# ray-project/anyscale-workshop-nyc-2023

Measured on NVIDIA H100. Metric: generated tokens/sec (and prompts/sec) FLAN-T5-base 512->128, higher is better.
Workload: dtype bf16

## Files before the change

### anyscale_workshop_nyc_2023_b200/_lib.py

```python
from __future__ import annotations

import ctypes as C
import os
import subprocess
from pathlib import Path

_HERE = Path(__file__).resolve().parent
LIB_PATH = _HERE / "libb200t5.so"
LIB_PATHS = {"bf16": LIB_PATH, "fp16": _HERE / "libb200t5_f16.so"}
CSRC = _HERE / "csrc"

OK, EINVAL, ENODEV, ECUDA, ESTATE, ENOMEM = 0, -1, -2, -3, -4, -5
DTYPE_BF16, DTYPE_F16, DTYPE_F32 = 0, 1, 2


class Config(C.Structure):
    _fields_ = [
        ("vocab_size", C.c_int32),
        ("d_model", C.c_int32),
        ("d_kv", C.c_int32),
        ("d_ff", C.c_int32),
        ("num_heads", C.c_int32),
        ("num_layers", C.c_int32),
        ("num_decoder_layers", C.c_int32),
# ... 3 lines not shown
        ("pad_token_id", C.c_int32),
        ("eos_token_id", C.c_int32),
        ("decoder_start_token_id", C.c_int32),
        ("is_gated_gelu", C.c_int32),
        ("scale_decoder_outputs", C.c_int32),
    ]


class GenParams(C.Structure):
    _fields_ = [
        ("max_new_tokens", C.c_int32),
        ("min_new_tokens", C.c_int32),
        ("eos_token_id", C.c_int32),
        ("pad_token_id", C.c_int32),
        ("decoder_start_token_id", C.c_int32),
        ("poll_interval", C.c_int32),
    ]


class Stats(C.Structure):
    _fields_ = [
        ("encoder_ms", C.c_float),
        ("decode_ms", C.c_float),
        ("decode_steps", C.c_int32),
        ("kernel_launches", C.c_int64),
        ("decode_algo_bytes", C.c_double),
        ("encoder_flops", C.c_double),
        ("xattn_kernel", C.c_int32),
        ("row_chains", C.c_int32),
    ]


_vp, _i, _i64p, _i32p = C.c_void_p, C.c_int, C.c_void_p, C.c_void_p

SIGNATURES = {
    "b200t5_create": (_i, [C.POINTER(Config), _i, C.POINTER(_vp)]),
    "b200t5_set_weight": (_i, [_vp, C.c_char_p, _vp, _i, C.POINTER(C.c_int64), _i]),
    "b200t5_finalize": (_i, [_vp]),
    "b200t5_destroy": (_i, [_vp]),
    "b200t5_last_error": (C.c_char_p, [_vp]),
    "b200t5_last_global_error": (C.c_char_p, []),
    "b200t5_generate": (_i, [_vp, _i64p, _i64p, _i, _i, C.POINTER(GenParams), _i64p, _i32p, _vp]),
    "b200t5_generate_host": (_i, [_vp, _i64p, _i64p, _i, _i, C.POINTER(GenParams), _i64p, _i32p]),
    "b200t5_generate_stream": (_i, [_vp, _i64p, _i64p, C.c_int64, _i, C.POINTER(GenParams), _i, _i, _i64p, _i32p]),
    "b200t5_get_stats": (_i, [_vp, C.POINTER(Stats)]),
    "b200t5_bench_cross_attn": (_i, [_vp, _i, _i, C.POINTER(C.c_float), C.POINTER(C.c_double), _vp]),
    "b200t5_set_option": (_i, [_vp, C.c_char_p, _i]),
    "b200t5_get_xattn_profile": (_i, [_vp, C.POINTER(C.c_double), C.POINTER(C.c_int64), C.POINTER(C.c_double), C.POINTER(C.c_double), C.POINTER(C.c_double)]),
    "b200t5_test_lm_argmax": (_i, [_i, _vp, _vp, _i, _i, _i, _i, _i, _i, _vp, _vp]),
    "b200t5_encode": (_i, [_vp, _i64p, _i64p, _i, _i, _vp, _vp]),
    "b200t5_decode_logits": (_i, [_vp, _i64p, _i64p, _i, _i, _i64p, _i, _vp, _vp]),
    "b200t5_relative_bucket": (_i, [_i, _i, _i, _i]),
    "b200t5_test_gemm": (_i, [_i, _vp, _vp, _vp, _i, _i, _i, _i, _i, _i, _vp]),
    "b200t5_test_gemm_splitk": (_i, [_i, _vp, _vp, _vp, _i, _i, _i, _i, _i, _i, _i, _vp, _i, _i, _vp]),
    "b200t5_test_ffo": (_i, [_i, _vp, _vp, _vp, _i, _i, _i, _i, _i, _i, _vp]),
    "b200t5_test_rmsnorm": (_i, [_i, _vp, _vp, _vp, _i, _i, C.c_float, _vp]),
    "b200t5_test_attn_decode": (_i, [_i, _i, _vp, _vp, _vp, _vp, _i, _i, _i, _vp, _vp, _i, _vp, _vp]),
    "b200t5_test_encoder_attn": (_i, [_i, _vp, _vp, _vp, _vp, _vp, _i, _i, _i, _i, _vp]),
    "b200t5_test_geglu": (_i, [_i, _vp, _vp, _vp, C.c_int64, _i, _vp]),
    "b200t5_version": (C.c_char_p, []),
}

_libs = {}


def build(force: bool = False) -> Path:
    for path in LIB_PATHS.values():
        if force and path.exists():
            path.unlink()
    proc = subprocess.run(["make", "-j2", "-C", str(CSRC)], capture_output=True, text=True)
    if proc.returncode != 0 or not all(path.exists() for path in LIB_PATHS.values()):
        raise RuntimeError(f"building libb200t5.so / libb200t5_f16.so failed:\n{proc.stdout}\n{proc.stderr}")
    return LIB_PATH


def load(flavour: str = "bf16") -> C.CDLL:
    if flavour in _libs:
        return _libs[flavour]
    path = LIB_PATHS[flavour]
    if not path.exists():
        raise RuntimeError(
            f"{path} is missing: run `make -C {CSRC}` (or __graft_entry__.build()). "
            "There is no CPU or PyTorch fallback for the CUDA path."
        )
    lib = C.CDLL(str(path), mode=getattr(os, "RTLD_NOW", 2))
    for name, (res, args) in SIGNATURES.items():
        try:
            fn = getattr(lib, name)
        except AttributeError as e:
            raise RuntimeError(f"{path.name} does not export {name}") from e
        fn.restype = res
        fn.argtypes = args
    _libs[flavour] = lib
    return lib


def last_error(handle=None, lib=None) -> str:
    lib = lib or load()
    msg = lib.b200t5_last_error(handle) if handle else lib.b200t5_last_global_error()
    return (msg or b"").decode("utf-8", "replace")


class B200T5Error(RuntimeError):
    def __init__(self, code: int, msg: str):
        super().__init__(f"libb200t5 error {code}: {msg}")
        self.code = code
# ... 6 lines not shown
```

### anyscale_workshop_nyc_2023_b200/csrc/b200t5.cu

```cuda
#include <cuda.h>
#include <cuda_bf16.h>
#include <cuda_fp16.h>
#include <cuda_runtime.h>
#include <math.h>
#include <stdarg.h>
#include <stdio.h>
#include <string.h>

#include <map>
#include <memory>
#include <string>
#include <vector>

#include "../../include/b200t5.h"
#include "attention_decode.cuh"
#include "attention_cross_stream.cuh"
#include "attention_encoder.cuh"
#include "elementwise.cuh"
#include "gemm.cuh"
#include "gemm_splitk.cuh"
#include "gemm_2cta.cuh"

using namespace b200;

// ... 198 lines not shown
  cudaGraphExec_t gexec8 = nullptr;
  long long g_eos = -1, g_pad = -1;
  int g_min_new = -1;
  long long* h_ids = nullptr;
  long long* h_mask = nullptr;
  long long* h_out = nullptr;
  int* h_len = nullptr;
  DecodeState* h_state = nullptr;
  ~Plan() {
    if (gexec) cudaGraphExecDestroy(gexec);
    if (graph) cudaGraphDestroy(graph);
    if (gexec8) cudaGraphExecDestroy(gexec8);
    if (graph8) cudaGraphDestroy(graph8);
    if (h_ids) cudaFreeHost(h_ids);
    if (h_mask) cudaFreeHost(h_mask);
    if (h_out) cudaFreeHost(h_out);
    if (h_len) cudaFreeHost(h_len);
    if (h_state) cudaFreeHost(h_state);
    if (h_cu) cudaFreeHost(h_cu);
    if (h_unf) cudaFreeHost(h_unf);
    if (h_admit) cudaFreeHost(h_admit);
  }
};

struct b200t5_ctx {
  Cfg c;
  int device = 0;
  int num_sms = 132;
  bool finalized = false;
  int ffo_k = 0;
  char err[512] = "";
  std::map<std::string, std::unique_ptr<DevBuf>> raw;
  std::map<std::string, std::unique_ptr<DevBuf>> raw_f32;
  std::map<std::string, std::vector<int64_t>> raw_shape;
  DevBuf shared, lm_head, enc_final_ln, dec_final_ln, enc_relbias, dec_relbias, wcrosskv;
  CUtensorMap tm_lm, tm_crosskv, tm2_crosskv;
  std::vector<float> enc_relbias_h, dec_relbias_h;
  std::vector<EncLayerW> enc;
  std::vector<DecLayerW> dec;
  std::unique_ptr<Plan> plan;
  cudaStream_t cap_stream = nullptr, exec_stream = nullptr, enc_stream = nullptr;
  cudaEvent_t enc_done_ev = nullptr, admitted_ev = nullptr;
  bool admit_overlap = true;
  cudaEvent_t ev[4] = {nullptr, nullptr, nullptr, nullptr};
  bool ev_valid = false;
  int pow_mode = 0;
  bool use_pdl = true;
  GeluLut gelu_lut{nullptr, 0, 0};
  struct SkChoice {
    int bn, split;
  };
  bool pack_rows = true;
  bool use_2cta = true;
  bool self_block = true;
  int xattn_mode = 2;
  int xs_stages = 5;
  bool xs_late_pdl = true;
  bool xs_l2_prefetch = false;
  bool xattn_serialize = false;
  std::vector<cudaEvent_t> xattn_ev;
  bool profile_xattn = false;
  int small_prio = 0;
  bool sk_on = true;
  int sk_stages64 = 0, sk_stages128 = 0;
  SkChoice sk_qkv{64, 2}, sk_proj{64, 4}, sk_wi{128, 2}, sk_ffo{64, 4};
  int chains_override = 0;
  cudaStream_t chain_streams[kMaxChains] = {};
  cudaEvent_t chain_ev[kMaxChains + 1] = {};
  int64_t launches = 0;
  int last_steps = 0;
  double last_decode_bytes = 0, last_enc_flops = 0;
};

static int fail(b200t5_ctx* h, int code, const char* fmt, ...) {
  char buf[512];
  va_list ap;
  va_start(ap, fmt);
  vsnprintf(buf, sizeof(buf), fmt, ap);
  va_end(ap);
  if (h) snprintf(h->err, sizeof(h->err), "%s", buf);
  snprintf(g_err, sizeof(g_err), "%s", buf);
  return code;
}

static int check_device(b200t5_ctx* h, int device) {
  int n = 0;
  cudaError_t e = cudaGetDeviceCount(&n);
  if (e != cudaSuccess || n <= 0)
    return fail(h, B200T5_ENODEV, "no CUDA device available (%s); libb200t5 has no CPU fallback",
                e == cudaSuccess ? "count=0" : cudaGetErrorString(e));
  if (device < 0 || device >= n) return fail(h, B200T5_EINVAL, "device %d out of range (%d devices)", device, n);
  cudaDeviceProp p;
  CU_OK(h, cudaGetDeviceProperties(&p, device));
  if (p.major != 9)
    return fail(h, B200T5_ENODEV, "device %d is sm_%d%d; libb200t5 is built for sm_90a only", device, p.major, p.minor);
  CU_OK(h, cudaSetDevice(device));
  return p.multiProcessorCount;
}

extern "C" int b200t5_relative_bucket(int rel, int bidirectional, int num_buckets, int max_distance) {
  int ret = 0, n;
  if (bidirectional) {
    num_buckets /= 2;
    if (rel > 0) ret += num_buckets;
    n = rel < 0 ? -rel : rel;
  } else {
    n = rel < 0 ? -rel : 0;
  }
  const int max_exact = num_buckets / 2;
  if (n < max_exact) return ret + n;
  const float ratio = static_cast<float>(n) / static_cast<float>(max_exact);
  const float denom = static_cast<float>(log(static_cast<double>(max_distance) / static_cast<double>(max_exact)));
  const float scaled = logf(ratio) / denom * static_cast<float>(num_buckets - max_exact);
  int large = max_exact + static_cast<int>(scaled);
  if (large > num_buckets - 1) large = num_buckets - 1;
  return ret + large;
}

static cudaError_t run_gemm(b200t5_ctx* h, const GemmOp& g, const void* ep, cudaStream_t s, bool pdl = false) {
  h->launches++;
  switch (g.kind) {
    case G_STORE256:
      return launch_gemm<256, EpiStore>(g.tmA, g.tmB, g.M, g.N, g.K, g.m_fastest, *static_cast<const EpiStore::Params*>(ep), h->num_sms, s, pdl);
    case G_RES256:
      return launch_gemm<256, EpiResidual>(g.tmA, g.tmB, g.M, g.N, g.K, g.m_fastest, *static_cast<const EpiResidual::Params*>(ep), h->num_sms, s, pdl);
    case G_GEGLU256:
      return launch_gemm<256, EpiGeglu>(g.tmA, g.tmB, g.M, g.N, g.K, g.m_fastest, *static_cast<const EpiGeglu::Params*>(ep), h->num_sms, s, pdl);
    case G_CROSSKV256:
      return launch_gemm<256, EpiCrossKV>(g.tmA, g.tmB, g.M, g.N, g.K, g.m_fastest, *static_cast<const EpiCrossKV::Params*>(ep), h->num_sms, s, pdl);
    case G_QKVDEC64:
      return launch_gemm<64, EpiQkvDecode>(g.tmA, g.tmB, g.M, g.N, g.K, g.m_fastest, *static_cast<const EpiQkvDecode::Params*>(ep), h->num_sms, s, pdl);
    case G_STORE32:
      return launch_gemm<32, EpiStore>(g.tmA, g.tmB, g.M, g.N, g.K, g.m_fastest, *static_cast<const EpiStore::Params*>(ep), h->num_sms, s, pdl);
    case G_RES32:
      return launch_gemm<32, EpiResidual>(g.tmA, g.tmB, g.M, g.N, g.K, g.m_fastest, *static_cast<const EpiResidual::Params*>(ep), h->num_sms, s, pdl);
    case G_GEGLU64:
      return launch_gemm<64, EpiGeglu>(g.tmA, g.tmB, g.M, g.N, g.K, g.m_fastest, *static_cast<const EpiGeglu::Params*>(ep), h->num_sms, s, pdl);
    case G_ARGMAX128:
      return launch_gemm<128, EpiArgmax>(g.tmA, g.tmB, g.M, g.N, g.K, g.m_fastest, *static_cast<const EpiArgmax::Params*>(ep), h->num_sms, s, pdl);
    case G_LOGITS128:
      return launch_gemm<128, EpiStoreF32>(g.tmA, g.tmB, g.M, g.N, g.K, g.m_fastest, *static_cast<const EpiStoreF32::Params*>(ep), h->num_sms, s, pdl);
  }
  return cudaErrorInvalidValue;
}

template <class Epi>
static cudaError_t run_gemm_2cta(b200t5_ctx* h, const CUtensorMap& tmA, const CUtensorMap& tmB, int M, int N, int K,
                                 const typename Epi::Params& ep, cudaStream_t s) {
  h->launches++;
  return launch_gemm_2cta<Epi>(tmA, tmB, M, N, K, ep, h->num_sms, s);
}

template <class Epi>
static cudaError_t run_gemm_sk(b200t5_ctx* h, const b200t5_ctx::SkChoice& ch, const CUtensorMap& tmA,
                               const CUtensorMap& tmB, int M, int N, int K, const typename Epi::Params& ep,
                               cudaStream_t s, bool pdl) {
  h->launches++;
  const int split = splitk_factor(K, ch.split);
  if (ch.bn == 128) return launch_gemm_splitk<128, Epi>(tmA, tmB, M, N, K, split, ep, s, pdl, 0, h->sk_stages128);
  return launch_gemm_splitk<64, Epi>(tmA, tmB, M, N, K, split, ep, s, pdl, 0, h->sk_stages64);
}

static cudaError_t run_ffo_2cta(b200t5_ctx* h, const CUtensorMap& tmA, const CUtensorMap& tmB, int M, int N,
                                const EpiResidual::Params& ep, cudaStream_t s) {
  h->launches++;
  return launch_gemm_2cta<EpiResidual, B200T5_F16 != 0>(tmA, tmB, M, N, h->ffo_k, ep, h->num_sms, s, B200T5_F16 ? h->ffo_k / 64 : 0);
}
static cudaError_t run_ffo_sk(b200t5_ctx* h, const b200t5_ctx::SkChoice& ch, const CUtensorMap& tmA, const CUtensorMap& tmB,
                              int M, int N, const EpiResidual::Params& ep, cudaStream_t s, bool pdl) {
  h->launches++;
  constexpr bool tf = B200T5_F16 != 0;
  const int split = splitk_factor(h->ffo_k, ch.split, tf ? kBK / 2 : kBK);
  const int akb = tf ? h->ffo_k / 64 : 0;
  if (ch.bn == 128) return launch_gemm_splitk<128, EpiResidual, tf>(tmA, tmB, M, N, h->ffo_k, split, ep, s, pdl, akb, h->sk_stages128);
  return launch_gemm_splitk<64, EpiResidual, tf>(tmA, tmB, M, N, h->ffo_k, split, ep, s, pdl, akb, h->sk_stages64);
}

static cudaError_t run_rmsnorm(b200t5_ctx* h, const res_t* x, const act_t* w, act_t* y, int M, int d, float eps,
                               cudaStream_t s, bool pdl = false) {
  if (h) h->launches++;
  const int wpb = 8;
  const int grid = (M + wpb - 1) / wpb;
  if (d <= 1024) return launch_kernel(rmsnorm_kernel<4>, dim3(grid), dim3(wpb * 32), 0, s, pdl, x, w, y, M, d, eps);
  if (d <= 4096) return launch_kernel(rmsnorm_kernel<16>, dim3(grid), dim3(wpb * 32), 0, s, pdl, x, w, y, M, d, eps);
  return cudaErrorInvalidValue;
}

static cudaError_t init_kernel_attrs() {
  cudaError_t e;
#define PREP(BN, EPI)                         \
  if ((e = prepare_gemm<BN, EPI>()) != cudaSuccess) return e;
  PREP(256, EpiStore) PREP(256, EpiResidual) PREP(256, EpiGeglu) PREP(256, EpiCrossKV) PREP(64, EpiQkvDecode)
  PREP(32, EpiStore) PREP(32, EpiResidual) PREP(64, EpiGeglu) PREP(128, EpiArgmax) PREP(128, EpiStoreF32)
  PREP(64, EpiStore) PREP(128, EpiStore)
#undef PREP
  if ((e = prepare_gemm_2cta<EpiStore>()) != cudaSuccess) return e;
  if ((e = prepare_gemm_2cta<EpiResidual>()) != cudaSuccess) return e;
  if ((e = prepare_gemm_2cta<EpiGeglu>()) != cudaSuccess) return e;
  if ((e = prepare_gemm_2cta<EpiCrossKV>()) != cudaSuccess) return e;
#define PREPSK(BN, EPI) \
  if ((e = prepare_gemm_splitk<BN, EPI>()) != cudaSuccess) return e;
  PREPSK(64, EpiStore) PREPSK(128, EpiStore) PREPSK(64, EpiResidual) PREPSK(128, EpiResidual)
  PREPSK(64, EpiQkvDecode) PREPSK(128, EpiQkvDecode) PREPSK(64, EpiGeglu) PREPSK(128, EpiGeglu)
#undef PREPSK
  if ((e = prepare_gemm_2cta<EpiResidual, B200T5_F16 != 0>()) != cudaSuccess) return e;
  if ((e = prepare_gemm_splitk<64, EpiResidual, B200T5_F16 != 0>()) != cudaSuccess) return e;
  if ((e = prepare_gemm_splitk<128, EpiResidual, B200T5_F16 != 0>()) != cudaSuccess) return e;
  if ((e = cudaFuncSetAttribute(self_attn_decode_warp_kernel, cudaFuncAttributeMaxDynamicSharedMemorySize,
                                kSelfWarpsPerCta * 4096 * 4)) != cudaSuccess)
    return e;
  if ((e = cudaFuncSetAttribute(attn_cross_stream_kernel, cudaFuncAttributeMaxDynamicSharedMemorySize,
                                static_cast<int>(XsSmem::bytes(kXsMaxStages, 4096)))) != cudaSuccess)
    return e;
  return cudaFuncSetAttribute(encoder_attn_kernel, cudaFuncAttributeMaxDynamicSharedMemorySize, 96 * 1024);
}

struct GeluLutOwner {
  DevBuf table;
  GeluLut lut{nullptr, 0, 0};
  int pow_mode = -1;
};
static GeluLutOwner g_gelu;

[[maybe_unused]] static int ensure_gelu_lut(b200t5_ctx* h, int pow_mode, GeluLut* out) {
  if (g_gelu.lut.table && g_gelu.pow_mode == pow_mode) {
    *out = g_gelu.lut;
    return B200T5_OK;
  }
  DevBuf full;
  CU_OK(h, full.alloc(65536 * 2));
  build_gelu_table_kernel<<<256, 256>>>(full.as<uint16_t>(), pow_mode);
  CU_OK(h, cudaGetLastError());
  std::vector<uint16_t> t(65536);
  CU_OK(h, cudaMemcpy(t.data(), full.p, 65536 * 2, cudaMemcpyDeviceToHost));
  auto half_bits = [](uint16_t xb) {
    uint32_t u = static_cast<uint32_t>(xb) << 16;
    float f;
    memcpy(&f, &u, 4);
    f *= 0.5f;
    memcpy(&u, &f, 4);
    u += 0x7FFFu + ((u >> 16) & 1u);
    return static_cast<uint16_t>(u >> 16);
  };
  int lo = 0;
  while (lo < 0x7F80 && t[lo] == half_bits(static_cast<uint16_t>(lo)) && t[0x8000 | lo] == half_bits(static_cast<uint16_t>(0x8000 | lo))) ++lo;
  int hi = 0x7F80;
  while (hi > lo && t[hi - 1] == static_cast<uint16_t>(hi - 1) && t[0x8000 | (hi - 1)] == 0x8000) --hi;
  const int n = hi - lo;
  if (n < 0 || 2 * n * 2 > kEpiSmemBytes) return fail(h, B200T5_ECUDA, "gelu table window [%#x,%#x) does not fit the epilogue scratch", lo, hi);
  std::vector<uint16_t> compact(((static_cast<size_t>(2) * (n > 0 ? n : 1) + 7) / 8) * 8 + 8, 0);
  for (int i = 0; i < n; ++i) {
    compact[i] = t[lo + i];
    compact[n + i] = t[0x8000 | (lo + i)];
  }
  CU_OK(h, g_gelu.table.alloc(compact.size() * 2));
  CU_OK(h, cudaMemcpy(g_gelu.table.p, compact.data(), compact.size() * 2, cudaMemcpyHostToDevice));
  g_gelu.lut = GeluLut{g_gelu.table.as<uint16_t>(), lo, hi};
  g_gelu.pow_mode = pow_mode;
  *out = g_gelu.lut;
  return B200T5_OK;
}

extern "C" const char* b200t5_version(void) {
  return B200T5_F16 ? "b200t5 0.1 fp16 (sm_90a, wgmma/TMA)" : "b200t5 0.1 (sm_90a, wgmma/TMA)";
}
extern "C" const char* b200t5_last_global_error(void) { return g_err; }
extern "C" const char* b200t5_last_error(b200t5_handle h) { return h ? h->err : g_err; }

extern "C" int b200t5_create(const b200t5_config* cfg, int device, b200t5_handle* out) {
  if (!cfg || !out) return fail(nullptr, B200T5_EINVAL, "null argument");
  *out = nullptr;
  if (cfg->d_kv != 64) return fail(nullptr, B200T5_EINVAL, "d_kv=%d unsupported (kernels are specialised for 64)", cfg->d_kv);
  if (!cfg->is_gated_gelu) return fail(nullptr, B200T5_EINVAL, "only feed_forward_proj='gated-gelu' (T5 v1.1 / FLAN-T5) is supported");
  if (cfg->scale_decoder_outputs) return fail(nullptr, B200T5_EINVAL, "scale_decoder_outputs (tied-embedding T5 v1.0) is not supported");
  if (cfg->d_model % 8 || cfg->d_ff % 32 || cfg->d_model > 4096 || cfg->vocab_size < 2 || cfg->num_heads < 1 ||
      cfg->num_layers < 1 || cfg->num_decoder_layers < 1)
    return fail(nullptr, B200T5_EINVAL, "unsupported shape: d_model=%d d_ff=%d vocab=%d", cfg->d_model, cfg->d_ff, cfg->vocab_size);
  int sms = check_device(nullptr, device);
  if (sms < 0) return sms;
  b200t5_ctx* h = new (std::nothrow) b200t5_ctx();
  if (!h) return fail(nullptr, B200T5_ENOMEM, "out of host memory");
  h->c = Cfg{cfg->vocab_size, cfg->d_model, cfg->d_ff, cfg->num_heads, cfg->num_heads * 64, cfg->num_layers,
             cfg->num_decoder_layers, cfg->relative_attention_num_buckets, cfg->relative_attention_max_distance,
             cfg->layer_norm_epsilon, cfg->pad_token_id, cfg->eos_token_id, cfg->decoder_start_token_id};
  h->device = device;
  h->num_sms = sms;
  h->enc.resize(h->c.Le);
  h->dec.resize(h->c.Ld);
  const char* pm = getenv("B200T5_POW_MODE");
  h->pow_mode = pm ? atoi(pm) : 0;
  const char* pdl_env = getenv("B200T5_PDL");
  h->use_pdl = pdl_env ? atoi(pdl_env) != 0 : true;
  if (const char* pr_env = getenv("B200T5_PRIO")) h->small_prio = atoi(pr_env);
  if (const char* pk_env = getenv("B200T5_PACK")) h->pack_rows = atoi(pk_env) != 0;
  if (const char* tc_env = getenv("B200T5_2CTA")) h->use_2cta = atoi(tc_env) != 0;
  if (const char* sf_env = getenv("B200T5_SELF")) h->self_block = strcmp(sf_env, "warp") != 0;
  if (const char* xa_env = getenv("B200T5_XATTN")) h->xattn_mode = strcmp(xa_env, "ldg") == 0 ? 0 : strcmp(xa_env, "stream") == 0 ? 1 : 2;
  if (const char* xs_env = getenv("B200T5_XS_STAGES")) {
    const int v = atoi(xs_env);
    if (v >= 2 && v <= kXsMaxStages) h->xs_stages = v;
  }
  if (const char* lp_env = getenv("B200T5_XS_LATE_PDL")) h->xs_late_pdl = atoi(lp_env) != 0;
  if (const char* se_env = getenv("B200T5_XS_SERIALIZE")) h->xattn_serialize = atoi(se_env) != 0;
  if (const char* pf_env = getenv("B200T5_XS_L2PF")) h->xs_l2_prefetch = atoi(pf_env) != 0;
  if (const char* sk_env = getenv("B200T5_SK")) {
    int v[8];
    const int n = sscanf(sk_env, "%d,%d,%d,%d,%d,%d,%d,%d", &v[0], &v[1], &v[2], &v[3], &v[4], &v[5], &v[6], &v[7]);
    if (n == 1 && v[0] == 0) h->sk_on = false;
    if (n == 8) {
      b200t5_ctx::SkChoice* dst[4] = {&h->sk_qkv, &h->sk_proj, &h->sk_wi, &h->sk_ffo};
      for (int i = 0; i < 4; ++i) {
        dst[i]->bn = v[2 * i] == 128 ? 128 : 64;
        dst[i]->split = v[2 * i + 1] >= 8 ? 8 : (v[2 * i + 1] >= 4 ? 4 : (v[2 * i + 1] >= 2 ? 2 : 1));
      }
    }
  }
  if (const char* st_env = getenv("B200T5_SK_STAGES")) {
    int a = 0, b = 0;
    if (sscanf(st_env, "%d,%d", &a, &b) == 2) {
      h->sk_stages64 = a;
      h->sk_stages128 = b;
    }
  }
  const char* ch_env = getenv("B200T5_CHAINS");
  h->chains_override = ch_env ? atoi(ch_env) : 0;
#if B200T5_F16
  h->use_2cta = h->pack_rows = true;
  if (!h->sk_on) {
    delete h;
    return fail(nullptr, B200T5_EINVAL, "B200T5_SK=0 is not available in the fp16 build");
  }
#endif
  if (const char* ao_env = getenv("B200T5_ADMIT_OVERLAP")) h->admit_overlap = atoi(ao_env) != 0;
  int prio_lo = 0, prio_hi = 0;
  cudaDeviceGetStreamPriorityRange(&prio_lo, &prio_hi);
  if (cudaStreamCreateWithFlags(&h->cap_stream, cudaStreamNonBlocking) != cudaSuccess ||
      cudaStreamCreateWithFlags(&h->exec_stream, cudaStreamNonBlocking) != cudaSuccess ||
      cudaStreamCreateWithPriority(&h->enc_stream, cudaStreamNonBlocking, prio_lo) != cudaSuccess ||
      cudaEventCreateWithFlags(&h->enc_done_ev, cudaEventDisableTiming) != cudaSuccess ||
      cudaEventCreateWithFlags(&h->admitted_ev, cudaEventDisableTiming) != cudaSuccess) {
    delete h;
    return fail(nullptr, B200T5_ECUDA, "cudaStreamCreate failed");
  }
  {
    cudaError_t ke = init_kernel_attrs();
    if (ke != cudaSuccess) {
      delete h;
      return fail(nullptr, B200T5_ECUDA, "kernel attribute setup failed: %s", cudaGetErrorString(ke));
// ... 1048 lines not shown
        cudaError_t e = launch_cross_attention(h, s, false, l, b0, nb, p.dq.as<act_t>() + static_cast<size_t>(b0) * c.I,
                                               p.dctx.as<act_t>() + static_cast<size_t>(b0) * c.I, p.extent.as<int>() + b0,
                                               p.key_ok.as<unsigned char>() + static_cast<size_t>(b0) * p.S, -1);
        if (e != cudaSuccess) le = e;
        ++launches;
      }
    }
  };
  sweep();
  CU_OK(h, le);
  cudaEvent_t e0 = nullptr, e1 = nullptr;
  struct EvGuard {
    cudaEvent_t &a, &b;
    ~EvGuard() {
      if (a) cudaEventDestroy(a);
      if (b) cudaEventDestroy(b);
    }
  } guard{e0, e1};
  CU_OK(h, cudaEventCreate(&e0));
  CU_OK(h, cudaEventCreate(&e1));
  CU_OK(h, cudaEventRecord(e0, s));
  for (int r = 0; r < reps; ++r) sweep();
  CU_OK(h, cudaEventRecord(e1, s));
  CU_OK(h, cudaEventSynchronize(e1));
  CU_OK(h, le);
  float ms = 0.f;
  CU_OK(h, cudaEventElapsedTime(&ms, e0, e1));
  CU_OK(h, cudaGetLastError());
  *avg_ms_per_launch = ms / (static_cast<float>(reps) * launches);
  std::vector<int> ext(p.B);
  CU_OK(h, cudaMemcpy(ext.data(), p.extent.p, p.B * 4, cudaMemcpyDeviceToHost));
  double sum_s = 0;
  for (int v : ext) sum_s += v;
  *bytes_per_launch = 2.0 * 2.0 * c.I * sum_s / (static_cast<double>(launches) / c.Ld);
  return B200T5_OK;
}

extern "C" int b200t5_set_option(b200t5_handle h, const char* name, int value) {
  if (!h || !name) return fail(h, B200T5_EINVAL, "null argument");
  const std::string n(name);
  if (n == "chains") h->chains_override = value < 0 ? 0 : value;
  else if (n == "xattn") h->xattn_mode = value < 0 || value > 2 ? 2 : value;
  else if (n == "xattn_stages") {
    if (value < 2 || value > kXsMaxStages) return fail(h, B200T5_EINVAL, "xattn_stages must be in [2, %d]", kXsMaxStages);
    h->xs_stages = value;
  } else if (n == "xattn_late_pdl") h->xs_late_pdl = value != 0;
  else if (n == "xattn_serialize") h->xattn_serialize = value != 0;
  else if (n == "xattn_l2pf") h->xs_l2_prefetch = value != 0;
  else if (n == "pdl") h->use_pdl = value != 0;
  else if (n == "admit_overlap") h->admit_overlap = value != 0;
  else if (n == "sk_stages64") h->sk_stages64 = value;
  else if (n == "sk_stages128") h->sk_stages128 = value;
  else if (n == "profile_xattn") h->profile_xattn = value != 0;
  else return fail(h, B200T5_EINVAL, "unknown option '%s'", name);
  CU_OK(h, cudaSetDevice(h->device));
  CU_OK(h, cudaDeviceSynchronize());
  h->plan.reset();
  return B200T5_OK;
}

extern "C" int b200t5_get_xattn_profile(b200t5_handle h, double* avg_us_per_launch, int64_t* launches, double* bytes_per_launch,
                                        double* busy_us_per_layer, double* bytes_per_layer) {
  if (!h || !avg_us_per_launch || !launches || !bytes_per_launch || !busy_us_per_layer || !bytes_per_layer)
    return fail(h, B200T5_EINVAL, "null argument");
  if (!h->plan || !h->profile_xattn) return fail(h, B200T5_ESTATE, "profiling is off (b200t5_set_option(h, \"profile_xattn\", 1), then generate)");
  CU_OK(h, cudaSetDevice(h->device));
  CU_OK(h, cudaDeviceSynchronize());
  Plan& p = *h->plan;
  const int n = h->c.Ld * p.n_chains;
  std::vector<unsigned long long> acc(static_cast<size_t>(n + h->c.Ld) * 2);
  CU_OK(h, cudaMemcpy(acc.data(), p.xs_acc.p, acc.size() * 8, cudaMemcpyDeviceToHost));
  unsigned long long ns = 0, cnt = 0, busy = 0, layers = 0;
  for (int i = 0; i < n; ++i) {
    ns += acc[2 * i];
    cnt += acc[2 * i + 1];
  }
  for (int l = 0; l < h->c.Ld; ++l) {
    busy += acc[2 * (n + l)];
    layers += acc[2 * (n + l) + 1];
  }
  *avg_us_per_launch = cnt ? static_cast<double>(ns) / static_cast<double>(cnt) / 1e3 : 0.0;
  *busy_us_per_layer = layers ? static_cast<double>(busy) / static_cast<double>(layers) / 1e3 : 0.0;
  *launches = static_cast<int64_t>(cnt);
  std::vector<int> ext(p.B);
  CU_OK(h, cudaMemcpy(ext.data(), p.extent.p, p.B * 4, cudaMemcpyDeviceToHost));
  double sum_s = 0;
  for (int v : ext) sum_s += v;
  *bytes_per_layer = 2.0 * 2.0 * h->c.I * sum_s;
  *bytes_per_launch = *bytes_per_layer / p.n_chains;
  return B200T5_OK;
}

extern "C" int b200t5_encode(b200t5_handle h, const int64_t* input_ids, const int64_t* attention_mask, int B, int S,
                             void* enc_out_bf16, void* stream) {
  TRY(validate(h, B, S, nullptr));
  if (!input_ids || !enc_out_bf16) return fail(h, B200T5_EINVAL, "null argument");
  CU_OK(h, cudaSetDevice(h->device));
  cudaStream_t s = static_cast<cudaStream_t>(stream);
  const int T = h->plan && h->plan->B == B && h->plan->S == S ? h->plan->Tmax : 1;
  TRY(ensure_plan(h, B, S, T));
  TRY(run_encoder(h, reinterpret_cast<const long long*>(input_ids), reinterpret_cast<const long long*>(attention_mask), s));
  if (h->plan->packed) {
    unpack_rows_kernel<<<dim3((S + 7) / 8, B), 256, 0, s>>>(h->plan->xn.as<act_t>(), h->plan->cu.as<int>(), static_cast<act_t*>(enc_out_bf16), S, h->c.d);
    CU_OK(h, cudaGetLastError());
  } else {
    CU_OK(h, cudaMemcpyAsync(enc_out_bf16, h->plan->xn.p, static_cast<size_t>(B) * S * h->c.d * 2, cudaMemcpyDeviceToDevice, s));
// ... 40 lines not shown
                                int pow_mode, void* stream) {
#if B200T5_F16
  return fail(nullptr, B200T5_EINVAL, "the single-kernel test hooks exist in the bf16 build only (libb200t5.so)");
#else
  const int sms = hook_device(device);
  if (sms < 0) return sms;
  if (K % 8) return fail(nullptr, B200T5_EINVAL, "K must be a multiple of 8");
  cudaStream_t s = static_cast<cudaStream_t>(stream);
  CUtensorMap ta, tb;
  if (!make_tmap(&ta, A, M, K, 128) || !make_tmap(&tb, W, N, K, bn == 512 ? 128 : bn)) return fail(nullptr, B200T5_ECUDA, "%s", g_err);
  b200t5_ctx dummy;
  dummy.num_sms = sms;
  cudaError_t e = cudaErrorInvalidValue;
  act_t* Cb = static_cast<act_t*>(C);
  if (bn == 512) {
    if (mode == 0) {
      EpiStore::Params ep{Cb, N};
      e = run_gemm_2cta<EpiStore>(&dummy, ta, tb, M, N, K, ep, s);
    } else if (mode == 1) {
      EpiResidual::Params ep{Cb, Cb, N};
      e = run_gemm_2cta<EpiResidual>(&dummy, ta, tb, M, N, K, ep, s);
    } else if (mode == 2) {
      GeluLut lut;
      int lrc = ensure_gelu_lut(nullptr, pow_mode, &lut);
      if (lrc != B200T5_OK) return lrc;
      EpiGeglu::Params ep{Cb, N / 2, lut};
      e = run_gemm_2cta<EpiGeglu>(&dummy, ta, tb, M, N, K, ep, s);
    }
    if (e != cudaSuccess) return fail(nullptr, B200T5_ECUDA, "test_gemm(pair, mode=%d): %s", mode, cudaGetErrorString(e));
    return B200T5_OK;
  }
  if (mode == 0) {
    EpiStore::Params ep{Cb, N};
    if (bn == 256) e = run_gemm(&dummy, mk(ta, tb, M, N, K, G_STORE256, 0), &ep, s);
    else if (bn == 32) e = run_gemm(&dummy, mk(ta, tb, M, N, K, G_STORE32, 1), &ep, s);
    else if (bn == 64) e = launch_gemm<64, EpiStore>(ta, tb, M, N, K, 0, ep, sms, s);
    else if (bn == 128) e = launch_gemm<128, EpiStore>(ta, tb, M, N, K, 0, ep, sms, s);
  } else if (mode == 1) {
    EpiResidual::Params ep{Cb, Cb, N};
    if (bn == 256) e = run_gemm(&dummy, mk(ta, tb, M, N, K, G_RES256, 0), &ep, s);
    else if (bn == 32) e = run_gemm(&dummy, mk(ta, tb, M, N, K, G_RES32, 1), &ep, s);
  } else if (mode == 2) {
    GeluLut lut;
    int lrc = ensure_gelu_lut(nullptr, pow_mode, &lut);
    if (lrc != B200T5_OK) return lrc;
    EpiGeglu::Params ep{Cb, N / 2, lut};
    if (bn == 256) e = run_gemm(&dummy, mk(ta, tb, M, N, K, G_GEGLU256, 0), &ep, s);
    else if (bn == 64) e = run_gemm(&dummy, mk(ta, tb, M, N, K, G_GEGLU64, 1), &ep, s);
  } else if (mode == 3) {
    EpiStoreF32::Params ep{static_cast<float*>(C), N};
    if (bn == 128) e = run_gemm(&dummy, mk(ta, tb, M, N, K, G_LOGITS128, 1), &ep, s);
  }
  if (e != cudaSuccess) return fail(nullptr, B200T5_ECUDA, "test_gemm(bn=%d, mode=%d): %s", bn, mode, cudaGetErrorString(e));
  return B200T5_OK;
#endif
}

extern "C" int b200t5_test_lm_argmax(int device, const void* x, const void* W, int M, int V, int K, int step, int eos,
                                     int min_new, int64_t* tokens, void* stream) {
  const int sms = hook_device(device);
  if (sms < 0) return sms;
  if (!x || !W || !tokens || M < 1 || V < 2 || K % 8 || step < 0) return fail(nullptr, B200T5_EINVAL, "test_lm_argmax: bad argument");
  cudaStream_t s = static_cast<cudaStream_t>(stream);
  CUtensorMap ta, tb;
  if (!make_tmap(&ta, x, M, K, 128) || !make_tmap(&tb, W, V, K, 128)) return fail(nullptr, B200T5_ECUDA, "%s", g_err);
  const int n_tiles = (V + 127) / 128, out_ld = step + 2;
  DevBuf pval, pidx, st, unf, out, len, xn, ext;
  if (pval.alloc(static_cast<size_t>(M) * n_tiles * 4) != cudaSuccess || pidx.alloc(static_cast<size_t>(M) * n_tiles * 4) != cudaSuccess ||
      st.alloc(sizeof(DecodeState)) != cudaSuccess || unf.alloc(static_cast<size_t>(M) * 4) != cudaSuccess ||
      out.alloc(static_cast<size_t>(M) * out_ld * 8) != cudaSuccess || len.alloc(static_cast<size_t>(M) * 4) != cudaSuccess ||
      xn.alloc(static_cast<size_t>(M) * K * sizeof(res_t)) != cudaSuccess || ext.alloc(static_cast<size_t>(M) * 4) != cudaSuccess)
    return fail(nullptr, B200T5_ENOMEM, "test_lm_argmax: allocation failed");
  b200t5_ctx dummy;
  dummy.num_sms = sms;
  decode_init_kernel<<<M, 128, 0, s>>>(st.as<DecodeState>(), unf.as<int>(), out.as<long long>(), len.as<int>(), out_ld, M, 0, 0,
                                       static_cast<const act_t*>(W), xn.as<res_t>(), K);
  set_state_kernel<<<1, 1, 0, s>>>(st.as<DecodeState>(), step);
  EpiArgmax::Params ep{pval.as<float>(), pidx.as<int>(), n_tiles, &st.as<DecodeState>()->step, eos, min_new, 0};
  cudaError_t e = run_gemm(&dummy, mk(ta, tb, M, V, K, G_ARGMAX128, 1), &ep, s, false);
  if (e == cudaSuccess)
    e = launch_kernel(finalize_step_kernel, dim3(M), dim3(128), 0, s, false, pval.as<float>(), pidx.as<int>(), n_tiles, st.as<DecodeState>(),
                      unf.as<int>(), out.as<long long>(), len.as<int>(), out_ld, static_cast<long long>(-1), static_cast<long long>(0),
                      static_cast<const act_t*>(W), xn.as<res_t>(), K, ext.as<int>(), static_cast<int*>(nullptr),
                      static_cast<const int*>(nullptr), 1 << 30);
  if (e == cudaSuccess)
    e = cudaMemcpy2DAsync(tokens, 8, out.as<long long>() + step + 1, static_cast<size_t>(out_ld) * 8, 8, M, cudaMemcpyDeviceToDevice, s);
  if (e == cudaSuccess) e = cudaStreamSynchronize(s);
  if (e != cudaSuccess) return fail(nullptr, B200T5_ECUDA, "test_lm_argmax: %s", cudaGetErrorString(e));
  return B200T5_OK;
}

extern "C" int b200t5_test_gemm_splitk(int device, const void* A, const void* W, void* C, int M, int N, int K, int bn,
                                       int split, int mode, int pow_mode, void* aux, int Tmax, int step, void* stream) {
#if B200T5_F16
  return fail(nullptr, B200T5_EINVAL, "the single-kernel test hooks exist in the bf16 build only (libb200t5.so)");
#else
  const int sms = hook_device(device);
  if (sms < 0) return sms;
  if (K % 8) return fail(nullptr, B200T5_EINVAL, "K must be a multiple of 8");
  cudaStream_t s = static_cast<cudaStream_t>(stream);
  if ((bn != 64 && bn != 128) || (split != 1 && split != 2 && split != 4 && split != 8))
    return fail(nullptr, B200T5_EINVAL, "test_gemm_splitk: bn in {64,128}, split in {1,2,4,8}");
  CUtensorMap ta, tb;
  if (!make_tmap(&ta, A, M, K, 128) || !make_tmap(&tb, W, N, K, bn)) return fail(nullptr, B200T5_ECUDA, "%s", g_err);
  b200t5_ctx dummy;
  dummy.num_sms = sms;
// ... 159 lines not shown
```

### anyscale_workshop_nyc_2023_b200/csrc/gemm_2cta.cuh

```cuda
#pragma once
#include "gemm.cuh"

namespace b200 {

constexpr int k2ctaBN = 256;
constexpr int k2ctaBox = 128;

template <class Epi, bool kTf32 = false>
cudaError_t prepare_gemm_2cta() {
  return prepare_gemm<k2ctaBN, Epi, kTf32, k2ctaBox>();
}

template <class Epi, bool kTf32 = false>
cudaError_t launch_gemm_2cta(const CUtensorMap& tmA, const CUtensorMap& tmB, int M, int N, int K,
                             const typename Epi::Params& ep, int num_sms, cudaStream_t stream, int a_kblocks = 0) {
  return launch_gemm<k2ctaBN, Epi, kTf32, k2ctaBox>(tmA, tmB, M, N, K, 0, ep, num_sms, stream, false, a_kblocks);
}

}
```

### include/b200t5.h

```cpp
#ifndef B200T5_H_
#define B200T5_H_

#include <stdint.h>

#ifdef __cplusplus
extern "C" {
#endif

#define B200T5_OK 0
#define B200T5_EINVAL (-1)
#define B200T5_ENODEV (-2)
#define B200T5_ECUDA (-3)
#define B200T5_ESTATE (-4)
#define B200T5_ENOMEM (-5)

#define B200T5_DTYPE_BF16 0
#define B200T5_DTYPE_F16 1
#define B200T5_DTYPE_F32 2

typedef struct b200t5_ctx* b200t5_handle;

typedef struct b200t5_config {
  int32_t vocab_size;
  int32_t d_model;
// ... 15 lines not shown
typedef struct b200t5_gen_params {
  int32_t max_new_tokens;
  int32_t min_new_tokens;
  int32_t eos_token_id;
  int32_t pad_token_id;
  int32_t decoder_start_token_id;
  int32_t poll_interval;
} b200t5_gen_params;

typedef struct b200t5_stats {
  float encoder_ms;
  float decode_ms;
  int32_t decode_steps;
  int64_t kernel_launches;
  double decode_algo_bytes;
  double encoder_flops;
  int32_t xattn_kernel;
  int32_t row_chains;
} b200t5_stats;

int b200t5_create(const b200t5_config* cfg, int device, b200t5_handle* out);
int b200t5_set_weight(b200t5_handle h, const char* name, const void* dev_ptr, int dtype, const int64_t* shape,
                      int ndim);
int b200t5_finalize(b200t5_handle h);
int b200t5_destroy(b200t5_handle h);
const char* b200t5_last_error(b200t5_handle h);
const char* b200t5_last_global_error(void);

int b200t5_generate(b200t5_handle h, const int64_t* input_ids, const int64_t* attention_mask, int B, int S,
                    const b200t5_gen_params* params, int64_t* out_ids, int32_t* out_len, void* stream);
int b200t5_generate_host(b200t5_handle h, const int64_t* input_ids, const int64_t* attention_mask, int B, int S,
                         const b200t5_gen_params* params, int64_t* out_ids, int32_t* out_len);
int b200t5_generate_stream(b200t5_handle h, const int64_t* input_ids, const int64_t* attention_mask, int64_t N, int S,
                           const b200t5_gen_params* params, int pool, int admit_min, int64_t* out_ids,
                           int32_t* out_len);
int b200t5_get_stats(b200t5_handle h, b200t5_stats* out);

int b200t5_bench_cross_attn(b200t5_handle h, int reps, int rows_per_launch, float* avg_ms_per_launch,
                            double* bytes_per_launch, void* stream);
int b200t5_set_option(b200t5_handle h, const char* name, int value);
int b200t5_get_xattn_profile(b200t5_handle h, double* avg_us_per_launch, int64_t* launches, double* bytes_per_launch,
                             double* busy_us_per_layer, double* bytes_per_layer);
int b200t5_test_lm_argmax(int device, const void* x, const void* W, int M, int V, int K, int step, int eos, int min_new,
                          int64_t* tokens, void* stream);

int b200t5_encode(b200t5_handle h, const int64_t* input_ids, const int64_t* attention_mask, int B, int S,
                  void* enc_out_bf16, void* stream);
int b200t5_decode_logits(b200t5_handle h, const int64_t* input_ids, const int64_t* attention_mask, int B, int S,
                         const int64_t* decoder_input_ids, int T, float* logits, void* stream);
int b200t5_relative_bucket(int relative_position, int bidirectional, int num_buckets, int max_distance);

int b200t5_test_gemm(int device, const void* A, const void* W, void* C, int M, int N, int K, int bn, int mode,
                     int pow_mode, void* stream);
int b200t5_test_gemm_splitk(int device, const void* A, const void* W, void* C, int M, int N, int K, int bn, int split,
                            int mode, int pow_mode, void* aux, int Tmax, int step, void* stream);
int b200t5_test_ffo(int device, const void* A, const void* W, void* R, int M, int N, int F, int kernel, int bn, int split,
                    void* stream);
int b200t5_test_rmsnorm(int device, const void* x, const void* w, void* y, int M, int d, float eps, void* stream);
int b200t5_test_attn_decode(int device, int self, const void* q, const void* K, const void* V, void* ctx, int B,
                            int H, int Tk, const int32_t* extent, const uint8_t* key_ok, int step,
                            const float* dist_bias, void* stream);
int b200t5_test_encoder_attn(int device, const void* qkv, void* ctx, const float* rel_bias, const uint8_t* key_ok,
                             const int32_t* extent, int B, int S, int H, int impl, void* stream);
int b200t5_test_geglu(int device, const void* gate, const void* up, void* out, int64_t n, int pow_mode,
                      void* stream);

const char* b200t5_version(void);

#ifdef __cplusplus
}
#endif
#endif
```

Before: 80280.

## Add warp-specialized persistent encoder GEMM with staged epilogue overlap

Adds a persistent warp-specialized GEMM for encoder projections. One TMA producer warp, two WGMMA consumer warpgroups and three dedicated epilogue warps share work through a shared-memory staging buffer, so each tile's epilogue overlaps the next tile's main loop. It is enabled by default for the 2-CTA-path encoder GEMMs and the bf16 FFN output GEMM, and can be switched off by env var or option. The cost is a smaller 3-stage ring plus a staging buffer, and a narrow epilogue warp set that may itself become the bottleneck.

```diff
diff --git a/anyscale_workshop_nyc_2023_b200/_lib.py b/anyscale_workshop_nyc_2023_b200/_lib.py
--- a/anyscale_workshop_nyc_2023_b200/_lib.py
+++ b/anyscale_workshop_nyc_2023_b200/_lib.py
@@ -79,6 +79,7 @@
     "b200t5_decode_logits": (_i, [_vp, _i64p, _i64p, _i, _i, _i64p, _i, _vp, _vp]),
     "b200t5_relative_bucket": (_i, [_i, _i, _i, _i]),
     "b200t5_test_gemm": (_i, [_i, _vp, _vp, _vp, _i, _i, _i, _i, _i, _i, _vp]),
+    "b200t5_test_enc_gemm": (_i, [_i, _vp, _vp, _vp, _i, _i, _i, _i, _i, _i, _vp, _vp, _i, _i, _i, _vp]),
     "b200t5_test_gemm_splitk": (_i, [_i, _vp, _vp, _vp, _i, _i, _i, _i, _i, _i, _i, _vp, _i, _i, _vp]),
     "b200t5_test_ffo": (_i, [_i, _vp, _vp, _vp, _i, _i, _i, _i, _i, _i, _vp]),
     "b200t5_test_rmsnorm": (_i, [_i, _vp, _vp, _vp, _i, _i, C.c_float, _vp]),
diff --git a/anyscale_workshop_nyc_2023_b200/csrc/b200t5.cu b/anyscale_workshop_nyc_2023_b200/csrc/b200t5.cu
--- a/anyscale_workshop_nyc_2023_b200/csrc/b200t5.cu
+++ b/anyscale_workshop_nyc_2023_b200/csrc/b200t5.cu
@@ -274,6 +274,7 @@
   };
   bool pack_rows = true;
   bool use_2cta = true;
+  bool enc_gemm_ws = true;
   bool self_block = true;
   int xattn_mode = 2;
   int xs_stages = 5;
@@ -370,6 +371,7 @@
 static cudaError_t run_gemm_2cta(b200t5_ctx* h, const CUtensorMap& tmA, const CUtensorMap& tmB, int M, int N, int K,
                                  const typename Epi::Params& ep, cudaStream_t s) {
   h->launches++;
+  if (h->enc_gemm_ws) return launch_gemm_enc_ws<Epi>(tmA, tmB, M, N, K, ep, h->num_sms, s);
   return launch_gemm_2cta<Epi>(tmA, tmB, M, N, K, ep, h->num_sms, s);
 }
 
@@ -386,6 +388,7 @@
 static cudaError_t run_ffo_2cta(b200t5_ctx* h, const CUtensorMap& tmA, const CUtensorMap& tmB, int M, int N,
                                 const EpiResidual::Params& ep, cudaStream_t s) {
   h->launches++;
+  if (!B200T5_F16 && h->enc_gemm_ws) return launch_gemm_enc_ws<EpiResidual>(tmA, tmB, M, N, h->ffo_k, ep, h->num_sms, s);
   return launch_gemm_2cta<EpiResidual, B200T5_F16 != 0>(tmA, tmB, M, N, h->ffo_k, ep, h->num_sms, s, B200T5_F16 ? h->ffo_k / 64 : 0);
 }
 static cudaError_t run_ffo_sk(b200t5_ctx* h, const b200t5_ctx::SkChoice& ch, const CUtensorMap& tmA, const CUtensorMap& tmB,
@@ -420,6 +423,10 @@
   if ((e = prepare_gemm_2cta<EpiResidual>()) != cudaSuccess) return e;
   if ((e = prepare_gemm_2cta<EpiGeglu>()) != cudaSuccess) return e;
   if ((e = prepare_gemm_2cta<EpiCrossKV>()) != cudaSuccess) return e;
+  if ((e = prepare_gemm_enc_ws<EpiStore>()) != cudaSuccess) return e;
+  if ((e = prepare_gemm_enc_ws<EpiResidual>()) != cudaSuccess) return e;
+  if ((e = prepare_gemm_enc_ws<EpiGeglu>()) != cudaSuccess) return e;
+  if ((e = prepare_gemm_enc_ws<EpiCrossKV>()) != cudaSuccess) return e;
 #define PREPSK(BN, EPI) \
   if ((e = prepare_gemm_splitk<BN, EPI>()) != cudaSuccess) return e;
   PREPSK(64, EpiStore) PREPSK(128, EpiStore) PREPSK(64, EpiResidual) PREPSK(128, EpiResidual)
@@ -516,6 +523,7 @@
   if (const char* pr_env = getenv("B200T5_PRIO")) h->small_prio = atoi(pr_env);
   if (const char* pk_env = getenv("B200T5_PACK")) h->pack_rows = atoi(pk_env) != 0;
   if (const char* tc_env = getenv("B200T5_2CTA")) h->use_2cta = atoi(tc_env) != 0;
+  if (const char* eg_env = getenv("B200T5_ENC_GEMM")) h->enc_gemm_ws = atoi(eg_env) != 0;
   if (const char* sf_env = getenv("B200T5_SELF")) h->self_block = strcmp(sf_env, "warp") != 0;
   if (const char* xa_env = getenv("B200T5_XATTN")) h->xattn_mode = strcmp(xa_env, "ldg") == 0 ? 0 : strcmp(xa_env, "stream") == 0 ? 1 : 2;
   if (const char* xs_env = getenv("B200T5_XS_STAGES")) {
@@ -1670,6 +1678,7 @@
   else if (n == "sk_stages64") h->sk_stages64 = value;
   else if (n == "sk_stages128") h->sk_stages128 = value;
   else if (n == "profile_xattn") h->profile_xattn = value != 0;
+  else if (n == "enc_gemm") h->enc_gemm_ws = value != 0;
   else return fail(h, B200T5_EINVAL, "unknown option '%s'", name);
   CU_OK(h, cudaSetDevice(h->device));
   CU_OK(h, cudaDeviceSynchronize());
@@ -1816,6 +1825,47 @@
     if (bn == 128) e = run_gemm(&dummy, mk(ta, tb, M, N, K, G_LOGITS128, 1), &ep, s);
   }
   if (e != cudaSuccess) return fail(nullptr, B200T5_ECUDA, "test_gemm(bn=%d, mode=%d): %s", bn, mode, cudaGetErrorString(e));
+  return B200T5_OK;
+#endif
+}
+
+extern "C" int b200t5_test_enc_gemm(int device, const void* A, const void* W, void* C, int M, int N, int K, int kernel,
+                                    int mode, int pow_mode, const int* row_b, const int* row_s, int B, int H, int S,
+                                    void* stream) {
+#if B200T5_F16
+  return fail(nullptr, B200T5_EINVAL, "the single-kernel test hooks exist in the bf16 build only (libb200t5.so)");
+#else
+  const int sms = hook_device(device);
+  if (sms < 0) return sms;
+  if (K % 8) return fail(nullptr, B200T5_EINVAL, "K must be a multiple of 8");
+  if (kernel != 0 && kernel != 1) return fail(nullptr, B200T5_EINVAL, "test_enc_gemm: kernel in {0, 1}");
+  if (mode == 3 && (H < 1 || S < 1 || B < 1 || N % (H * 64) || (!row_b) != (!row_s) || (!row_b && M != B * S)))
+    return fail(nullptr, B200T5_EINVAL, "test_enc_gemm: bad cross-KV arguments");
+  cudaStream_t s = static_cast<cudaStream_t>(stream);
+  CUtensorMap ta, tb;
+  if (!make_tmap(&ta, A, M, K, 128) || !make_tmap(&tb, W, N, K, k2ctaBox)) return fail(nullptr, B200T5_ECUDA, "%s", g_err);
+  b200t5_ctx dummy;
+  dummy.num_sms = sms;
+  dummy.enc_gemm_ws = kernel == 1;
+  cudaError_t e = cudaErrorInvalidValue;
+  act_t* Cb = static_cast<act_t*>(C);
+  if (mode == 0) {
+    EpiStore::Params ep{Cb, N};
+    e = run_gemm_2cta<EpiStore>(&dummy, ta, tb, M, N, K, ep, s);
+  } else if (mode == 1) {
+    EpiResidual::Params ep{Cb, Cb, N};
+    e = run_gemm_2cta<EpiResidual>(&dummy, ta, tb, M, N, K, ep, s);
+  } else if (mode == 2) {
+    GeluLut lut;
+    int lrc = ensure_gelu_lut(nullptr, pow_mode, &lut);
+    if (lrc != B200T5_OK) return lrc;
+    EpiGeglu::Params ep{Cb, N / 2, lut};
+    e = run_gemm_2cta<EpiGeglu>(&dummy, ta, tb, M, N, K, ep, s);
+  } else if (mode == 3) {
+    EpiCrossKV::Params ep{Cb, B, H, S, row_b, row_s};
+    e = run_gemm_2cta<EpiCrossKV>(&dummy, ta, tb, M, N, K, ep, s);
+  }
+  if (e != cudaSuccess) return fail(nullptr, B200T5_ECUDA, "test_enc_gemm(kernel=%d, mode=%d): %s", kernel, mode, cudaGetErrorString(e));
   return B200T5_OK;
 #endif
 }
diff --git a/anyscale_workshop_nyc_2023_b200/csrc/gemm_2cta.cuh b/anyscale_workshop_nyc_2023_b200/csrc/gemm_2cta.cuh
--- a/anyscale_workshop_nyc_2023_b200/csrc/gemm_2cta.cuh
+++ b/anyscale_workshop_nyc_2023_b200/csrc/gemm_2cta.cuh
@@ -17,4 +17,221 @@
   return launch_gemm<k2ctaBN, Epi, kTf32, k2ctaBox>(tmA, tmB, M, N, K, 0, ep, num_sms, stream, false, a_kblocks);
 }
 
-}
+constexpr int kEncWsThreads = 384;
+constexpr int kEncWsEpiThreads = 96;
+constexpr int kEncWsEpiWarp0 = 9;
+
+struct EncWsCfg {
+  static constexpr int kBN = k2ctaBN;
+  static constexpr int kStages = 3;
+  static constexpr int kABytes = kBM * kBK * 2;
+  static constexpr int kBBytes = kBN * kBK * 2;
+  static constexpr int kStageBytes = kABytes + kBBytes;
+  static constexpr int kRingBytes = kStages * kStageBytes;
+  static constexpr int kStagingBytes = kBM * kBN * 2;
+  static constexpr int kSmemBytes = kRingBytes + kStagingBytes + 1024  + 256  + kEpiSmemBytes;
+  static_assert(kSmemBytes <= 227 * 1024, "shared memory");
+};
+
+DEVINL uint32_t enc_stg_unit(int r, int u) {
+  const int f = ((u >> 3) & 3) ^ (((r & 1) << 1) | ((r >> 1) & 1) | (r & 4));
+  return static_cast<uint32_t>(r * 512 + ((u ^ f) << 4));
+}
+
+DEVINL void enc_stage_act(uint32_t stg, int row0, const float (&acc)[k2ctaBN / 2]) {
+  const int t = threadIdx.x & 127;
+  const int r = row0 + 16 * (t >> 5) + ((t & 31) >> 2);
+  const uint32_t w = 4u * (t & 3);
+#pragma unroll
+  for (int j = 0; j < k2ctaBN / 8; ++j) {
+    asm volatile("st.shared.b32 [%0], %1;" ::"r"(stg + enc_stg_unit(r, j) + w), "r"(pack_act2(acc[4 * j], acc[4 * j + 1])) : "memory");
+    asm volatile("st.shared.b32 [%0], %1;" ::"r"(stg + enc_stg_unit(r + 8, j) + w), "r"(pack_act2(acc[4 * j + 2], acc[4 * j + 3])) : "memory");
+  }
+}
+
+DEVINL void enc_stg_ld_chunk(uint32_t stg, int r, int u0, uint32_t (&acc)[32]) {
+#pragma unroll
+  for (int g = 0; g < 4; ++g) {
+    uint32_t w[4];
+    asm volatile("ld.shared.v4.b32 {%0, %1, %2, %3}, [%4];"
+                 : "=r"(w[0]), "=r"(w[1]), "=r"(w[2]), "=r"(w[3])
+                 : "r"(stg + enc_stg_unit(r, u0 + g))
+                 : "memory");
+#pragma unroll
+    for (int k = 0; k < 4; ++k) {
+      acc[8 * g + 2 * k] = __float_as_uint(act_lo(w[k]));
+      acc[8 * g + 2 * k + 1] = __float_as_uint(act_hi(w[k]));
+    }
+  }
+}
+
+template <class Epi>
+DEVINL void enc_ws_drain(const typename Epi::Params& p, uint32_t stg, int m0, int M, int n_tile, int N,
+                         const uint8_t* es, int e, uint64_t* full, uint32_t parity) {
+  if constexpr (Epi::kPaired) {
+    mbar_wait(full, parity);
+#pragma unroll 1
+    for (int i = e; i < kBM * 4; i += kEncWsEpiThreads) {
+      const int r = i >> 2, c = i & 3;
+      const int m = m0 + r, f0 = n_tile * (k2ctaBN / 2) + c * 32;
+      uint32_t g[32], u[32];
+      enc_stg_ld_chunk(stg, r, 4 * c, g);
+      enc_stg_ld_chunk(stg, r, 16 + 4 * c, u);
+      if (m < M && f0 < p.F) Epi::chunk2(p, g, u, m, f0, es);
+    }
+  } else {
+    constexpr int kItems = kBM * 8;
+    typename Epi::ChunkPre pre[2];
+    const int n_base = n_tile * k2ctaBN;
+    if (m0 + (e >> 3) < M && n_base + (e & 7) * 32 < N) Epi::chunk_pre(p, m0 + (e >> 3), n_base + (e & 7) * 32, N, pre[0]);
+    mbar_wait(full, parity);
+#pragma unroll 1
+    for (int i = e; i < kItems; i += 2 * kEncWsEpiThreads) {
+#pragma unroll
+      for (int v = 0; v < 2; ++v) {
+        const int it = i + v * kEncWsEpiThreads;
+        if (it < kItems) {
+          const int nx = it + kEncWsEpiThreads;
+          if (nx < kItems && m0 + (nx >> 3) < M && n_base + (nx & 7) * 32 < N)
+            Epi::chunk_pre(p, m0 + (nx >> 3), n_base + (nx & 7) * 32, N, pre[(v + 1) & 1]);
+          const int r = it >> 3, c = it & 7;
+          const int m = m0 + r, n0 = n_base + c * 32;
+          uint32_t acc[32];
+          enc_stg_ld_chunk(stg, r, 4 * c, acc);
+          if (m < M && n0 < N) Epi::chunk(p, acc, m, n0, N, es, pre[v]);
+        }
+      }
+    }
+  }
+}
+
+template <class Epi>
+__global__ void __launch_bounds__(kEncWsThreads, 1)
+gemm_enc_ws_kernel(const __grid_constant__ CUtensorMap tmA, const __grid_constant__ CUtensorMap tmB, int M, int N, int K,
+                   typename Epi::Params ep) {
+  using Cfg = EncWsCfg;
+  constexpr int BN = Cfg::kBN;
+  extern __shared__ uint8_t smem_raw[];
+  uint8_t* smem = reinterpret_cast<uint8_t*>((reinterpret_cast<uintptr_t>(smem_raw) + 1023) & ~uintptr_t(1023));
+  const uint32_t stg = smem_u32(smem + Cfg::kRingBytes);
+  uint64_t* bars = reinterpret_cast<uint64_t*>(smem + Cfg::kRingBytes + Cfg::kStagingBytes);
+  uint64_t* full = bars;
+  uint64_t* empty = bars + Cfg::kStages;
+  uint64_t* stg_full = bars + 2 * Cfg::kStages;
+  uint64_t* stg_empty = stg_full + 1;
+  uint8_t* epi_smem = smem + Cfg::kRingBytes + Cfg::kStagingBytes + 256;
+
+  const int warp = threadIdx.x >> 5;
+  const int lane = threadIdx.x & 31;
+  const int tiles_m = (M + kBM - 1) / kBM;
+  const int tiles_n = (N + BN - 1) / BN;
+  const int num_tiles = tiles_m * tiles_n;
+  const int kblocks = (K + kBK - 1) / kBK;
+
+  pdl_launch_dependents();
+  if (threadIdx.x == 0) {
+    for (int i = 0; i < Cfg::kStages; ++i) {
+      mbar_init(&full[i], 1);
+      mbar_init(&empty[i], 2);
+    }
+    mbar_init(stg_full, kGemmConsumers);
+    mbar_init(stg_empty, kEncWsEpiThreads);
+    mbar_fence_init();
+  }
+  __syncthreads();
+
+  if (warp == 8) {
+    if (lane == 0) {
+      tma_prefetch_desc(&tmA);
+      tma_prefetch_desc(&tmB);
+      if (static_cast<int>(blockIdx.x) < num_tiles) {
+        const TileCoord tc0 = tile_coord(blockIdx.x, tiles_m, tiles_n, 0);
+        for (int kb = 0; kb < kblocks; ++kb)
+          for (int p = 0; p < BN / k2ctaBox; ++p) tma_prefetch_l2_2d(&tmB, kb * kBK, tc0.n_tile * BN + p * k2ctaBox);
+      }
+      pdl_wait();
+      int stage = 0;
+      uint32_t phase = 0;
+      for (int tile = blockIdx.x; tile < num_tiles; tile += gridDim.x) {
+        const TileCoord tc = tile_coord(tile, tiles_m, tiles_n, 0);
+        const int m0 = tc.m_tile * kBM, n0 = tc.n_tile * BN;
+        for (int kb = 0; kb < kblocks; ++kb) {
+          mbar_wait(&empty[stage], phase ^ 1u);
+          uint8_t* sA = smem + stage * Cfg::kStageBytes;
+          uint8_t* sB = sA + Cfg::kABytes;
+          mbar_arrive_expect_tx(&full[stage], Cfg::kStageBytes);
+          tma_load_2d(sA, &tmA, &full[stage], kb * kBK, m0);
+#pragma unroll
+          for (int p = 0; p < BN / k2ctaBox; ++p) tma_load_2d(sB + p * k2ctaBox * 128, &tmB, &full[stage], kb * kBK, n0 + p * k2ctaBox);
+          if (++stage == Cfg::kStages) {
+            stage = 0;
+            phase ^= 1u;
+          }
+        }
+      }
+    }
+  } else if (warp >= kEncWsEpiWarp0) {
+    const int e = threadIdx.x - kEncWsEpiWarp0 * 32;
+    Epi::prologue(ep, epi_smem, e, kEncWsEpiThreads);
+    pdl_wait();
+    uint32_t sphase = 0;
+    for (int tile = blockIdx.x; tile < num_tiles; tile += gridDim.x) {
+      const TileCoord tc = tile_coord(tile, tiles_m, tiles_n, 0);
+      enc_ws_drain<Epi>(ep, stg, tc.m_tile * kBM, M, tc.n_tile, N, epi_smem, e, stg_full, sphase);
+      mbar_arrive(stg_empty);
+      sphase ^= 1u;
+    }
+  } else {
+    const int wg = warp >> 2;
+    int stage = 0;
+    uint32_t phase = 0, sphase = 0;
+    for (int tile = blockIdx.x; tile < num_tiles; tile += gridDim.x) {
+      float acc[BN / 2];
+#pragma unroll
+      for (int i = 0; i < BN / 2; ++i) acc[i] = 0.f;
+      int prev = -1;
+      for (int kb = 0; kb < kblocks; ++kb) {
+        mbar_wait(&full[stage], phase);
+        const uint32_t a_addr = smem_u32(smem + stage * Cfg::kStageBytes) + wg * 64 * 128;
+        wgmma_fence_acc(acc);
+        wgmma_fence();
+        wgmma_kblock<BN, false>(acc, a_addr, smem_u32(smem + stage * Cfg::kStageBytes + Cfg::kABytes));
+        wgmma_commit();
+        wgmma_wait<1>();
+        wgmma_fence_acc(acc);
+        if (prev >= 0 && (threadIdx.x & 127) == 0) mbar_arrive(&empty[prev]);
+        prev = stage;
+        if (++stage == Cfg::kStages) {
+          stage = 0;
+          phase ^= 1u;
+        }
+      }
+      wgmma_wait<0>();
+      wgmma_fence_acc(acc);
+      if (prev >= 0 && (threadIdx.x & 127) == 0) mbar_arrive(&empty[prev]);
+      mbar_wait(stg_empty, sphase ^ 1u);
+      enc_stage_act(stg, wg * 64, acc);
+      mbar_arrive(stg_full);
+      sphase ^= 1u;
+    }
+  }
+}
+
+template <class Epi>
+cudaError_t prepare_gemm_enc_ws() {
+  return cudaFuncSetAttribute(gemm_enc_ws_kernel<Epi>, cudaFuncAttributeMaxDynamicSharedMemorySize, EncWsCfg::kSmemBytes);
+}
+
+template <class Epi>
+cudaError_t launch_gemm_enc_ws(const CUtensorMap& tmA, const CUtensorMap& tmB, int M, int N, int K,
+                               const typename Epi::Params& ep, int num_sms, cudaStream_t stream) {
+  if constexpr (std::is_same<Epi, EpiResidual>::value) {
+    if (!ep.round_acc) return cudaErrorInvalidValue;
+  }
+  const int tiles = ((M + kBM - 1) / kBM) * ((N + k2ctaBN - 1) / k2ctaBN);
+  const int grid = tiles < num_sms ? tiles : num_sms;
+  return launch_kernel(gemm_enc_ws_kernel<Epi>, dim3(grid), dim3(kEncWsThreads), EncWsCfg::kSmemBytes, stream, false,
+                       tmA, tmB, M, N, K, ep);
+}
+
+}
diff --git a/include/b200t5.h b/include/b200t5.h
--- a/include/b200t5.h
+++ b/include/b200t5.h
@@ -91,6 +91,8 @@
 
 int b200t5_test_gemm(int device, const void* A, const void* W, void* C, int M, int N, int K, int bn, int mode,
                      int pow_mode, void* stream);
+int b200t5_test_enc_gemm(int device, const void* A, const void* W, void* C, int M, int N, int K, int kernel, int mode,
+                         int pow_mode, const int* row_b, const int* row_s, int B, int H, int S, void* stream);
 int b200t5_test_gemm_splitk(int device, const void* A, const void* W, void* C, int M, int N, int K, int bn, int split,
                             int mode, int pow_mode, void* aux, int Tmax, int step, void* stream);
 int b200t5_test_ffo(int device, const void* A, const void* W, void* R, int M, int N, int F, int kernel, int bn, int split,
```

After: 82850 (median of 6 runs). 1.03x the previous value.
